# Suyashagarw/StreamOptima

Measured on AMD Instinct MI355X. Metric: encoded Mpixels/sec at 1080p & 4K, 1/2/4/8 GPUs; PSNR delta vs reference, higher is better.
Workload: dtype u8

## Files before the change

include/streamoptima.h:

```cpp
#ifndef STREAMOPTIMA_H
#define STREAMOPTIMA_H

#include <stddef.h>
#include <stdint.h>

#ifdef __cplusplus
extern "C" {
#endif

#define SO_OK 0
#define SO_E_INVALID (-1)
#define SO_E_UNSUPPORTED (-2)
#define SO_MAX_REF 4
#define SO_ABI_VERSION 1

int so_abi_version(void);
const char* so_last_error(void);

int so_me_full_search(const uint8_t* cur, const uint8_t* const* refs, int nref, int H,
                      int W, int bs, int sr, int32_t* out_best, int32_t* out_sub,
                      void* stream);

int so_inter_tq_recon(const uint8_t* cur, const uint8_t* const* refs, int nref, int H,
                      int W, int bs, const int32_t* best, const int32_t* sub, int qp_rd,
                      const int32_t* qp_row, int vbs, double lam, uint8_t* out_split,
                      int16_t* out_mv, int16_t* out_qtc, int32_t* out_tokens,
                      int32_t* out_mae_num, uint8_t* out_recon, int32_t* out_sse, void* stream);

size_t so_p_frame_scratch_elems(int H, int W, int bs, int vbs);

int so_encode_p_frame(const uint8_t* cur, const uint8_t* const* refs, int nref, int H,
                      int W, int bs, int sr, int qp_rd, const int32_t* qp_row, int vbs,
                      double lam, uint8_t* out_split, int16_t* out_mv, int16_t* out_qtc,
                      int32_t* out_tokens, int32_t* out_mae_num, uint8_t* out_recon,
                      int32_t* out_sse, int32_t* scratch, void* stream);

int so_encode_p_rows(const uint8_t* cur, const uint8_t* const* refs, int nref, int H, int W,
                     int bs, int sr, int by0, int by1, int qp_rd, const int32_t* qp_row,
                     int vbs, double lam, uint8_t* out_split, int16_t* out_mv,
                     int16_t* out_qtc, int32_t* out_tokens, int32_t* out_mae_num,
                     uint8_t* out_recon, int32_t* out_sse, int32_t* scratch, void* stream);

#define SO_OPT_RUN_2PASS_FUSED 1
#define SO_OPT_FASTME_SERIAL 2
#define SO_OPT_FASTME_SEGMENT 3
#define SO_OPT_FASTME_WARMUP 4
#define SO_OPT_COUNT_SAD_OPS 5
#define SO_OPT_TEST_LOSE_FLAG 6
#define SO_OPT_RUN_ZERO_SKIP 7
#define SO_OPT_RUN_TALL_TILES 8
int so_set_option(int option, int value);
int so_get_option(int option);

#define SO_P_RUN_TIMEOUT_WORD 32
#define SO_P_RUN_FALLBACK_WORD 64
#define SO_P_RUN_SAD_OPS_WORD 66
#define SO_P_RUN_TQ_FALLBACK_WORD 68
#define SO_P_RUN_STALE_WORD 33
#define SO_P_RUN_GAP_WORD 34
#define SO_P_RUN_DIAG_WORD 96
#define SO_P_RUN_DIAG_MAGIC 0x534F0001u
size_t so_p_run_workspace_elems(int H, int W);
int so_p_run_resident_workgroups(int vbs);
int so_p_run_mode_resident_workgroups(int mode, int vbs);
int so_p_run_tile_rows(int H, int W, int conc);
int so_encode_p_run(const uint8_t* const* curs, int nframes, const uint8_t* ref0, int H, int W,
                    int bs, int sr, int qp_rd, const int32_t* qp_row, int vbs, double lam,
                    uint8_t* const* out_split,
                    int16_t* const* out_mv, int16_t* const* out_qtc, int32_t* const* out_tokens,
                    int32_t* const* out_mae_num, uint8_t* const* out_recon, int32_t* const* out_sse,
                    uint32_t* workspace, void* stream);

int so_p_run_2pass_fused(int H, int W);

int so_encode_p_run_2pass(const uint8_t* const* curs, int nframes, const uint8_t* ref0, int H, int W,
                          int bs, int sr, int qp_rd, const int32_t* qp_row, const int32_t* roi,
                          int qp_lo, int qp_hi, uint8_t* const* out_split, int16_t* const* out_mv,
                          int16_t* const* out_qtc, int32_t* const* out_tokens,
                          int32_t* const* out_mae_num, uint8_t* const* out_recon,
                          int32_t* const* out_sse, int32_t* const* out_qp_map, uint32_t* workspace,
                          void* stream);

int so_encode_p_runs(const uint8_t* const* curs, int nframes, const uint8_t* const* refs,
// ... 273 lines not shown
```

streamoptima_amd/_lib.py:

```python
from __future__ import annotations

import ctypes
import os
import threading

import torch

from .build import LIB_PATH

_lock = threading.Lock()
_lib = None

SO_OK = 0
SO_E_INVALID = -1
SO_E_UNSUPPORTED = -2
MAX_REF = 4

_vp = ctypes.c_void_p
_i = ctypes.c_int
_d = ctypes.c_double
_sz = ctypes.c_size_t

_SIGS = {
    "so_abi_version": ([], _i),
# ... 79 lines not shown
    "so_pack_frames_huff": ([_i, _vp, _vp, _vp, _vp, _i, _i, _vp, _vp, ctypes.c_ulonglong, _vp, _vp], _i),
    "so_unpack_frames_huff": ([_i, _vp, _vp, _vp, _i, _i, _vp, _vp, _vp, _vp, _vp], _i),
    "so_pack_chroma_huff_bound": ([_i], _sz),
    "so_pack_chroma_frames_huff": ([_i, _vp, _vp, _i, _vp, _vp, ctypes.c_ulonglong, _vp, _vp], _i),
    "so_pack_chroma_frames_huff_after": ([_i, _vp, _vp, _i, _vp, _vp, _vp, ctypes.c_ulonglong, _vp, _vp], _i),
    "so_unpack_chroma_frames_huff": ([_i, _vp, _vp, _i, _vp, _vp, _vp, _vp], _i),
    "so_decode_p_frames": ([_i, _i, _vp, _vp, _i, _i, _i, _i, _vp, _vp, _vp, _i, _i, _vp, _vp, _vp, _vp, _vp], _i),
    "so_decode_chroma_frames": ([_i, _i, _vp, _vp, _vp, _i, _i, _i, _vp, _vp, _i, _vp, _vp, _i, _vp, _vp, _i, _i,
                                 _vp, _vp, _vp, _vp], _i),
    "so_decode_chroma_frames_ex": ([_i, _i, _vp, _vp, _vp, _i, _i, _i, _vp, _vp, _i, _vp, _vp, _i, _vp, _vp, _i, _i,
                                    _vp, _vp, _vp, _i, _vp], _i),
    "so_fme_plane_stride": ([_i, _i], _sz),
    "so_fme_workspace_bytes": ([_i, _i, _i], _sz),
    "so_fme_planes": ([_vp, _i, _i, _i, _vp, _vp], _i),
    "so_me_search_ex": ([_vp, _vp, _i, _i, _i, _i, _i, _i, _i, _i, _vp, _vp, _vp, _vp], _i),
    "so_encode_p_rows_ex": ([_vp, _vp, _i, _i, _i, _i, _i, _i, _i, _i, _vp, _vp, _i, _d, _i, _i, _i, _vp, _i,
                             _vp, _vp, _vp, _vp, _vp, _vp, _vp, _vp, _vp], _i),
    "so_inter_recon_ex": ([_vp, _i, _i, _i, _i, _i, _vp, _vp, _i, _i, _vp, _vp, _vp, _vp, _vp, _vp], _i),
    "so_encode_i_rows_ex": ([_vp, _i, _i, _i, _i, _i, _i, _i, _vp, _vp, _i, _d, _vp, _vp, _vp, _vp, _vp, _vp,
                             _vp, _vp, _vp], _i),
    "so_intra_recon_ex": ([_i, _i, _i, _i, _vp, _vp, _vp, _vp, _vp, _vp, _vp, _vp], _i),
    "so_qp_map": ([_vp, _i, _i, _i, _i, _i, _i, _vp, _vp, _i, _i, _vp, _vp], _i),
    "so_set_option": ([_i, _i], _i),
    "so_get_option": ([_i], _i),
}

ME_FULL, ME_FAST, ME_FAST_PAR = 0, 1, 2
REUSE_ME = 1
TOKENS_ONLY = 2
OPT_RUN_2PASS_FUSED, OPT_FASTME_SERIAL, OPT_FASTME_SEGMENT, OPT_FASTME_WARMUP, OPT_COUNT_SAD_OPS = 1, 2, 3, 4, 5
OPT_RUN_ZERO_SKIP = 7
OPT_RUN_TALL_TILES = 8
OPT_TEST_LOSE_FLAG = 6
COLOUR_MATRICES = {"bt601": 0, "bt709": 1}
COLOUR_LAYOUTS = {"hwc": 0, "chw": 1}

EXPORTED = tuple(_SIGS)


class HipPathError(RuntimeError):
    """Raised when the gfx950 library is unavailable or a kernel call fails."""


def load(path: str | None = None):
    global _lib
    with _lock:
        if _lib is not None:
            return _lib
        p = path or os.environ.get("SO_LIB_PATH") or LIB_PATH
        if not os.path.exists(p):
            raise HipPathError(
                f"{p} is missing: build it with `python -m streamoptima_amd.build` (hipcc, gfx950). "
                "There is no CPU fallback for the encode path.")
        lib = ctypes.CDLL(p)
        for name, (args, res) in _SIGS.items():
            if p != LIB_PATH and not hasattr(lib, name):
                continue
            fn = getattr(lib, name)
            fn.argtypes = args
            fn.restype = res
        if lib.so_abi_version() != 1:
            raise HipPathError("libstreamoptima_hip.so ABI mismatch")
        _lib = lib
        return lib


# ... 50 lines not shown
```

streamoptima_amd/csrc/so_capi.hip:

```cpp
#include <stdarg.h>
#include <stdio.h>
#include <stdlib.h>
#include <string.h>

#include <algorithm>
#include <atomic>
#include <vector>

#include <hip/hip_ext.h>

#include "so_chroma.h"
#include "so_colour.h"
#include "so_common.h"
#include "so_deblock.h"
#include "so_launch.h"
#include "so_packfmt.h"
#include "so_run.h"
#include "so_scale.h"

namespace so {

static thread_local char g_err[512] = "";

void set_error(const char* fmt, ...) {
    va_list ap;
    va_start(ap, fmt);
    vsnprintf(g_err, sizeof(g_err), fmt, ap);
    va_end(ap);
}

static std::atomic<int> g_opt[9] = {0, 1, 0, 32, 32, 0, 0, 0, -1};

int option(int id) {
    return (id > 0 && id < 9) ? g_opt[id].load(std::memory_order_relaxed) : 0;
}

#ifdef SO_AB
extern "C" int so_debug_ab_build(void) { return 1; }
#endif

static bool use_fused(int bs, int sr, int vbs, int nref) {
    if (bs != 16 || sr != 16 || vbs || nref != 1) return false;
#ifdef SO_AB
    const char* f = getenv("SO_FUSED");
    if (f && strcmp(f, "0") == 0) return false;
    const char* impl = getenv("SO_ME_IMPL");
    return impl == nullptr || impl[0] == 0;
#else
    return true;
#endif
}

static int check_vbs(const char* fn, int vbs, double lam) {
    if (vbs != 0 && vbs != 1) {
        set_error("%s: vbs must be 0 or 1", fn);
        return SO_E_INVALID;
    }
    if (vbs && !(lam >= 0.0 && lam < 1e300)) {
        set_error("%s: lambda %g (VBSEnable needs a finite lambda >= 0)", fn, lam);
        return SO_E_INVALID;
    }
    return SO_OK;
}

static int check_geom(const char* fn, int H, int W, int bs, int vbs) {
    if (bs != 16 && bs != 8) {
        set_error("%s: block_size %d not built (gfx950 kernels exist for 16 and 8)", fn, bs);
// ... 147 lines not shown
};

static int check_spans(const char* fn, std::vector<Span>& spans, bool dst_vs_dst) {
    std::sort(spans.begin(), spans.end(), [](const Span& a, const Span& b) { return a.lo < b.lo; });
    const Span *far_src = nullptr, *far_dst = nullptr;
    for (const Span& s : spans) {
        const Span* hit = nullptr;
        if (far_dst && s.lo < far_dst->hi && (!s.dst || dst_vs_dst)) hit = far_dst;
        if (!hit && s.dst && far_src && s.lo < far_src->hi) hit = far_src;
        if (hit) {
            set_error("%s: %s[%d] aliases %s[%d] (a destination overlaps a source or another destination)", fn,
                      s.what, s.frame, hit->what, hit->frame);
            return SO_E_INVALID;
        }
        const Span*& far = s.dst ? far_dst : far_src;
        if (!far || s.hi > far->hi) far = &s;
    }
    return SO_OK;
}

}

using namespace so;

extern "C" {

int so_abi_version(void) { return SO_ABI_VERSION; }

int so_set_option(int opt, int value) {
    const bool ok = (opt == SO_OPT_RUN_2PASS_FUSED || opt == SO_OPT_FASTME_SERIAL || opt == SO_OPT_COUNT_SAD_OPS ||
                     opt == SO_OPT_RUN_ZERO_SKIP)
                        ? (value == 0 || value == 1)
                    : opt == SO_OPT_RUN_TALL_TILES                               ? (value >= -1 && value <= 1)
                    : opt == SO_OPT_FASTME_SEGMENT                               ? value >= 1
                    : opt == SO_OPT_FASTME_WARMUP || opt == SO_OPT_TEST_LOSE_FLAG ? value >= 0
                                                                                 : false;
    if (!ok) {
        set_error("so_set_option: option %d value %d is unknown or out of range", opt, value);
        return SO_E_INVALID;
    }
    g_opt[opt].store(value, std::memory_order_relaxed);
    return SO_OK;
}

int so_get_option(int opt) { return option(opt); }

const char* so_last_error(void) { return g_err; }

int so_me_full_search(const uint8_t* cur, const uint8_t* const* refs, int nref, int H, int W, int bs,
                      int sr, int32_t* out_best, int32_t* out_sub, void* stream) {
    const char* fn = "so_me_full_search";
    SO_TRY(check_geom(fn, H, W, bs, out_sub != nullptr));
    SO_TRY(check_sr(fn, sr));
    SO_NEED(cur, fn);
    SO_NEED(out_best, fn);
    RefSet rs;
    SO_TRY(make_refs(fn, refs, nref, &rs));
    return me_launch(cur, rs, nref, H, W, bs, sr, 0, H / bs, out_best, out_sub, (hipStream_t)stream);
}

int so_inter_tq_recon(const uint8_t* cur, const uint8_t* const* refs, int nref, int H, int W, int bs,
                      const int32_t* best, const int32_t* sub, int qp_rd, const int32_t* qp_row, int vbs,
                      double lam, uint8_t* out_split, int16_t* out_mv, int16_t* out_qtc, int32_t* out_tokens,
                      int32_t* out_mae_num, uint8_t* out_recon, int32_t* out_sse, void* stream) {
    const char* fn = "so_inter_tq_recon";
    SO_TRY(check_geom(fn, H, W, bs, vbs));
// ... 1349 lines not shown
```

streamoptima_amd/csrc/so_intra.hip:

```cpp
#include "so_block.h"
#include "so_launch.h"

namespace so {

constexpr int kIntraMaxSr = 64;

SO_DEV uint32_t intra_key(int sad, int dx, int scan_rev) {
    return ((uint32_t)sad << 15) | ((uint32_t)(dx < 0 ? -dx : dx) << 8) | (uint32_t)scan_rev;
}

SO_DEV int canvas_at(const uint8_t* left , int sr, int col, int x0) {
    return col < x0 ? (int)left[col - (x0 - sr)] : 128;
}

template <int BS, bool VBS, int SRM = kIntraMaxSr>
__global__ void __launch_bounds__(256)
intra_tq_kernel(const uint8_t* __restrict__ cur, int H, int W, int by0, int nrows, int sr, int qp_rd,
                const int32_t* __restrict__ qp_row, const int32_t* __restrict__ qp_map, double lam,
                uint8_t* __restrict__ out_split,
                int16_t* __restrict__ out_mv, int16_t* __restrict__ out_qtc,
                int32_t* __restrict__ out_tokens, int32_t* __restrict__ out_mae,
                uint8_t* __restrict__ idres) {
    constexpr int G = BS, BPW = 256 / G, SB = BS / 2;
    constexpr int LDS_D = VBS ? 288 : BS * (BS + 1);
    __shared__ double ldsd[BPW * LDS_D];
    __shared__ uint8_t ldsf[VBS ? BPW * BS * BS : 1];
    __shared__ uint8_t ldsl[BPW * BS * SRM];
    const int tid = threadIdx.x, g = tid / G, l = tid % G;
    const int nbx = W / BS, nb = nbx * nrows;
    const int b = blockIdx.x * BPW + g;
    if (b >= nb) return;
    double* dl = ldsd + g * LDS_D;
    uint8_t* fl = ldsf + g * BS * BS;
    uint8_t* left = ldsl + g * BS * SRM;
    const int bx = b % nbx, by = by0 + b / nbx, x = bx * BS, y = by * BS;
    const int qpr = qp_map ? qp_map[(size_t)by * nbx + bx] : (qp_row ? qp_row[by] : qp_rd);

    uint8_t* lrow = left + l * SRM;
    if (BS == 16 && sr == 16 && x != 0) {
        *reinterpret_cast<uint4*>(lrow) = *reinterpret_cast<const uint4*>(cur + (size_t)(y + l) * W + x - 16);
    } else {
        for (int k = 0; k < sr; ++k) {
            const int col = x - sr + k;
            lrow[k] = col >= 0 ? cur[(size_t)(y + l) * W + col] : 0;
        }
    }
    int crow[BS];
    load_cur_row<BS>(cur, W, x, y + l, crow);
    wave_sync();

    int mv, sad;
    if (x == 0) {
        int s = 0;
#pragma unroll
        for (int c = 0; c < BS; ++c) s += abs(crow[c] - 128);
        sad = group_sum<G>(s);
        mv = -1;
    } else if (BS == 16 && sr == 16) {
        const uint8_t* rp = cur + (size_t)(y + l) * W + x;
        const uint4 lv = *reinterpret_cast<const uint4*>(rp - 16), cv = *reinterpret_cast<const uint4*>(rp);
        const uint32_t Z[9] = {lv.x, lv.y, lv.z, lv.w, 0x80808080u, 0x80808080u, 0x80808080u, 0x80808080u,
                               0x80808080u};
        const uint32_t C[4] = {cv.x, cv.y, cv.z, cv.w};
        uint32_t bestk = 0xFFFFFFFFu;
#pragma unroll
        for (int dx = -16; dx <= 0; ++dx) {
            const int off = 16 + dx, d = off >> 2, sh = off & 3;
            uint32_t srow = 0;
#pragma unroll
            for (int k = 0; k < 4; ++k)
                srow = __builtin_amdgcn_sad_u8(C[k], __builtin_amdgcn_alignbyte(Z[d + k + 1], Z[d + k], sh), srow);
            const int sfull = group_sum<G>((int)srow);
            const uint32_t key = ((uint32_t)sfull << 8) | (uint32_t)(-dx);
            bestk = key < bestk ? key : bestk;
        }
        sad = (int)(bestk >> 8);
        mv = -(int)(bestk & 0xFF);
    } else {
        uint32_t bestk = 0xFFFFFFFFu;
        for (int dxi = 0; dxi <= 2 * sr; ++dxi) {
            const int dx = dxi - sr;
            if (!(x + dx >= 0 && x + dx + BS <= W)) continue;
            int s = 0;
#pragma unroll
            for (int c = 0; c < BS; ++c) s += abs(crow[c] - canvas_at(lrow, sr, x + dx + c, x));
            s = group_sum<G>(s);
            const uint32_t k = intra_key(s, dx, 2 * sr - dxi);
            bestk = k < bestk ? k : bestk;
        }
        sad = (int)(bestk >> 15);
        mv = 2 * sr - (int)(bestk & 0xFF) - sr;
    }
    int res[BS];
#pragma unroll
    for (int c = 0; c < BS; ++c) res[c] = crow[c] - (x == 0 ? 128 : canvas_at(lrow, sr, x + mv + c, x));
    double tcd[BS];
    xform2d_rows<BS, false>(dl, l, res, tcd);
    int tc[BS], q[BS];
#pragma unroll
    for (int c = 0; c < BS; ++c) tc[c] = (int)__builtin_rint(tcd[c]);
    quant_row_i<BS>(tc, l, qp_rd, q);

    bool split = false;
    int mae_num = sad;
    const int j = l >> 2, r0 = l & 3;
    int smv = 0, stc[2][8], qs[2][8];
    if constexpr (VBS) {
        if (x != 0 && y != 0) {
            const int xs = x + (j & 1) * SB, oy = (j >> 1) * SB;
            int scur[2][8];
#pragma unroll
            for (int h = 0; h < 2; ++h) load_cur_row<8>(cur, W, xs, y + oy + r0 + 4 * h, scur[h]);
            int ssad;
            if (sr == 16) {
                uint32_t Zs[2][9], Cs[2][2];
#pragma unroll
                for (int h = 0; h < 2; ++h) {
                    const uint8_t* rp = cur + (size_t)(y + oy + r0 + 4 * h) * W + x;
                    const uint4 lv = *reinterpret_cast<const uint4*>(rp - 16);
                    const uint2 cv = *reinterpret_cast<const uint2*>(rp + (j & 1) * 8);
                    Zs[h][0] = lv.x; Zs[h][1] = lv.y; Zs[h][2] = lv.z; Zs[h][3] = lv.w;
                    Zs[h][4] = Zs[h][5] = Zs[h][6] = Zs[h][7] = Zs[h][8] = 0x80808080u;
                    Cs[h][0] = cv.x; Cs[h][1] = cv.y;
                }
                const int base = 16 + (j & 1) * 8;
                uint32_t bestk = 0xFFFFFFFFu;
#pragma unroll
                for (int dx = -16; dx <= 0; ++dx) {
                    const int off = base + dx;
                    const int d = off >> 2, sh = off & 3;
                    uint32_t srow = 0;
#pragma unroll
                    for (int h = 0; h < 2; ++h) {
                        uint32_t w0 = Zs[h][0], w1 = Zs[h][1], w2 = Zs[h][2];
// ... 31 lines not shown
                ssad = (int)(bestk >> 15);
                smv = 2 * sr - (int)(bestk & 0xFF) - sr;
            }
            int sres[2][8];
#pragma unroll
            for (int h = 0; h < 2; ++h) {
                const uint8_t* lr = left + (oy + r0 + 4 * h) * SRM;
#pragma unroll
                for (int c = 0; c < 8; ++c) sres[h][c] = scur[h][c] - canvas_at(lr, sr, xs + smv + c, x);
            }
            double std_[2][8];
            xform2d_sub<false>(dl, l, sres, std_);
            const int qpm1_rd = qp_rd > 0 ? qp_rd - 1 : qp_rd;
#pragma unroll
            for (int h = 0; h < 2; ++h) {
#pragma unroll
                for (int c = 0; c < 8; ++c) stc[h][c] = (int)__builtin_rint(std_[h][c]);
                quant_row<8>(stc[h], r0 + 4 * h, qpm1_rd, qs[h]);
            }
            const int tok_b = block_tokens<BS>(fl, l, q);
            const int tok_v = sub_tokens(fl, l, qs);
            int ssum = (r0 == 0) ? ssad : 0;
            ssum = group_sum<16>(ssum);
            const double mae_b = (double)sad / 256.0;
            const double mae_v = (double)ssum / 256.0;
            const double c_v = rd_cost(lam, 32 + 8 * tok_v, mae_v);
            const double c_b = rd_cost(lam, 8 + 8 * tok_b, mae_b);
            split = !(c_b < c_v);
            mae_num = ssum;
        }
    }

    int tok;
    uint8_t* rb = idres + (size_t)b * BS * BS;
    if (!split) {
        if (qpr != qp_rd) quant_row_i<BS>(tc, l, qpr, q);
        tok = block_tokens<BS>(fl, l, q);
        store_row_i16<BS>(out_qtc + (size_t)b * BS * BS + l * BS, q);
        int dq[BS];
        dequant_row_int<BS>(q, l, qpr, dq);
        double rd[BS];
        xform2d_rows<BS, true>(dl, l, dq, rd);
        int rr[BS];
#pragma unroll
        for (int c = 0; c < BS; ++c) rr[c] = (int)__builtin_rint(rd[c]);
        store_row_u8<BS>(rb, BS, 0, l, rr);
        for (int k = l; k < 4; k += G) out_mv[(size_t)b * 4 + k] = (int16_t)(k == 0 ? mv : 0);
    } else {
        if constexpr (VBS) {
            const int qpm1 = qpr > 0 ? qpr - 1 : qpr;
            const int qpm1_rd = qp_rd > 0 ? qp_rd - 1 : qp_rd;
            if (qpm1 != qpm1_rd)
#pragma unroll
                for (int h = 0; h < 2; ++h) quant_row<8>(stc[h], r0 + 4 * h, qpm1, qs[h]);
            tok = sub_tokens(fl, l, qs);
            int sdq[2][8];
#pragma unroll
            for (int h = 0; h < 2; ++h) {
                store_row_i16<8>(out_qtc + (size_t)b * BS * BS + j * 64 + (r0 + 4 * h) * 8, qs[h]);
                dequant_row<8>(qs[h], r0 + 4 * h, qpm1, sdq[h]);
            }
            double srd[2][8];
            xform2d_sub<true>(dl, l, sdq, srd);
#pragma unroll
            for (int h = 0; h < 2; ++h) {
                int rr[SB];
#pragma unroll
                for (int c = 0; c < SB; ++c) rr[c] = (int)__builtin_rint(srd[h][c]);
                store_row_u8<SB>(rb, BS, (j & 1) * SB, (j >> 1) * SB + r0 + 4 * h, rr);
            }
            if (r0 == 0) out_mv[(size_t)b * 4 + j] = (int16_t)smv;
        } else {
            tok = 0;
        }
    }
    if (l == 0) {
        out_split[b] = (uint8_t)split;
        out_tokens[b] = tok;
        out_mae[b] = mae_num;
    }
}

template <int BS, bool VBS>
__global__ void __launch_bounds__(256)
dequant_idct_kernel(int H, int W, int qp, const int32_t* __restrict__ qp_row, const int32_t* __restrict__ qp_map,
                    const uint8_t* __restrict__ split, const int16_t* __restrict__ qtc,
                    uint8_t* __restrict__ idres) {
    constexpr int G = BS, BPW = 256 / G;
    constexpr int LDS_D = VBS ? 288 : BS * (BS + 1);
    __shared__ double ldsd[BPW * LDS_D];
    const int tid = threadIdx.x, g = tid / G, l = tid % G;
    const int nbx = W / BS, nb = nbx * (H / BS);
    const int b = blockIdx.x * BPW + g;
    if (b >= nb) return;
    double* dl = ldsd + g * LDS_D;
    const int by = b / nbx;
    const int qpr = qp_map ? qp_map[b] : (qp_row ? qp_row[by] : qp);
    uint8_t* rb = idres + (size_t)b * BS * BS;
    if (!VBS || !split[b]) {
        int q[BS], dq[BS];
        load_row_i16<BS>(qtc + (size_t)b * BS * BS + l * BS, q);
        dequant_row<BS>(q, l, qpr, dq);
        double rd[BS];
        xform2d_rows<BS, true>(dl, l, dq, rd);
        int rr[BS];
#pragma unroll
        for (int c = 0; c < BS; ++c) rr[c] = (int)__builtin_rint(rd[c]);
        store_row_u8<BS>(rb, BS, 0, l, rr);
    } else if constexpr (VBS) {
        const int j = l >> 2, r0 = l & 3;
        const int qpm1 = qpr > 0 ? qpr - 1 : qpr;
        int sdq[2][8];
// ... 147 lines not shown
            const int bx = bx0 + s;
            if (bx < nbx) {
                const int x = bx * BS;
                int v = resc[s] + 128;
                const int src = x + c + dxc[s];
                if (x != 0 && src < x) v = resc[s] + vr[src & (RING - 1)];
                vr[(x + c) & (RING - 1)] = v;
                const int o = v & 255;
                if (act) {
                    orow[x + c] = (uint8_t)o;
                    const int d = curc[s] - o;
                    sse += d * d;
                }
            }
        }
    }
    if (out_sse) {
#pragma unroll
        for (int m = BS / 2; m >= 1; m >>= 1) sse += __shfl_xor(sse, m, 64);
        if (act && c == 0) out_sse[yl] = sse;
    }
}

template <int BS, int WPR>
__global__ void __launch_bounds__(64 * WPR)
intra_recon_scan_kernel(int W, int nrows_px, int by0, const uint8_t* __restrict__ split, const int16_t* __restrict__ mv,
                        const uint8_t* __restrict__ idres, const uint8_t* __restrict__ cur,
                        uint8_t* __restrict__ out_recon, int32_t* __restrict__ out_sse) {
    constexpr int NT = 64 * WPR, K = NT / BS, GPW = 64 / BS, SB = BS / 2, ND = BS / 4, TU = 4, U3 = 4;
    extern __shared__ __attribute__((aligned(16))) uint16_t slot[];
    __shared__ int ssum[WPR];
    const int tid = threadIdx.x, lane = tid & 63, wv = tid >> 6;
    const int k = tid / BS, c = tid - k * BS, g = k - wv * GPW;
    const int xcd = blockIdx.x & 7, kx = blockIdx.x >> 3;
    const int yl = (((kx / BS) << 3) + xcd) * BS + kx % BS;
    if (yl >= nrows_px) return;
    const int yy = by0 * BS + yl, byl = yl / BS, i = yl - byl * BS, nbx = W / BS;
    const int L = (nbx + K - 1) / K, j0 = k * L;
    const bool lower = i >= SB;
    uint32_t* const ev = reinterpret_cast<uint32_t*>(slot + (size_t)L * NT);
    uint8_t* const rowb = reinterpret_cast<uint8_t*>(ev + NT);
    for (int t0 = 0; t0 * NT < nbx; t0 += TU) {
        uint32_t rw[TU][ND], mw[TU][2], sp[TU];
#pragma unroll
        for (int t = 0; t < TU; ++t) {
            int jb = (t0 + t) * NT + tid;
            jb = jb < nbx ? jb : nbx - 1;
            const size_t b = (size_t)byl * nbx + jb;
            const uint32_t* rp = reinterpret_cast<const uint32_t*>(idres + b * BS * BS + i * BS);
#pragma unroll
            for (int d = 0; d < ND; ++d) rw[t][d] = rp[d];
            const uint2 m4 = *reinterpret_cast<const uint2*>(mv + b * 4);
            mw[t][0] = m4.x;
            mw[t][1] = m4.y;
            sp[t] = split[b];
        }
#pragma unroll
        for (int t = 0; t < TU; ++t) {
            const int jb = (t0 + t) * NT + tid;
            if (jb < nbx) {
                const uint32_t wlr = (sp[t] && lower) ? mw[t][1] : mw[t][0];
                const int dxl = (int)(int16_t)(wlr & 0xFFFF);
                const int dxr = sp[t] ? (int)(int16_t)(wlr >> 16) : dxl;
                const int kq = jb / L, s = jb - kq * L;
                uint32_t pk[BS / 2];
#pragma unroll
                for (int cc = 0; cc < BS; ++cc) {
                    const int rel = cc + (cc >= SB ? dxr : dxl);
                    const bool use = jb != 0 && rel < 0;
                    const uint32_t v = ((rw[t][cc >> 2] >> (8 * (cc & 3))) & 255u) | (use ? 256u : 0u) |
                                       ((uint32_t)((rel + BS) & (BS - 1)) << 9);
                    pk[cc >> 1] = (cc & 1) ? (pk[cc >> 1] | (v << 16)) : v;
                }
                uint4* dst = reinterpret_cast<uint4*>(slot + (size_t)s * NT + kq * BS);
#pragma unroll
                for (int q = 0; q < BS / 8; ++q) dst[q] = make_uint4(pk[4 * q], pk[4 * q + 1], pk[4 * q + 2], pk[4 * q + 3]);
            }
        }
    }
    __syncthreads();
    const int gbase = lane & ~(BS - 1);
    const int nvalid = nbx - j0 < L ? (nbx - j0 > 0 ? nbx - j0 : 0) : L;
    uint32_t w = (uint32_t)(c + 1) << 8;
    uint32_t in = slot[tid];
    for (int s = 0; s < nvalid; ++s) {
        const uint32_t cin = in;
        if (s + 1 < nvalid) in = slot[(s + 1) * NT + tid];
        const uint32_t gv = (uint32_t)__builtin_amdgcn_ds_bpermute((gbase + (int)(cin >> 9)) << 2, (int)w);
        const bool use = (cin & 256u) != 0u;
        w = ((cin + (use ? gv : 128u)) & 255u) | (use ? (gv & 0x1F00u) : 0u);
        slot[s * NT + tid] = (uint16_t)w;
    }
    uint32_t P = w;
#pragma unroll
    for (int gg = 1; gg < GPW; ++gg) {
        const uint32_t si = (w >> 8) & 31u;
        const uint32_t pg = (uint32_t)__builtin_amdgcn_ds_bpermute(((gg - 1) * BS + (int)(si ? si - 1 : 0)) << 2, (int)P);
        if (g == gg) P = ((w + (si ? pg : 0u)) & 255u) | (si ? (pg & 0x1F00u) : 0u);
    }
#pragma unroll
    for (int ww = 0; ww < WPR; ++ww) {
        if (wv == ww) {
            const uint32_t si = (P >> 8) & 31u;
            const uint32_t e = (ww > 0 && si) ? ev[(ww * GPW - 1) * BS + si - 1] : 0u;
            ev[tid] = (P + e) & 255u;
        }
        __syncthreads();
    }
    const uint32_t* const ein = ev + (k > 0 ? k - 1 : 0) * BS - 1;
    for (int s0 = 0; s0 < nvalid; s0 += U3) {
        uint32_t m[U3];
#pragma unroll
        for (int u = 0; u < U3; ++u) m[u] = s0 + u < nvalid ? slot[(s0 + u) * NT + tid] : 0u;
#pragma unroll
        for (int u = 0; u < U3; ++u) {
// ... 5 lines not shown
    __syncthreads();
    const uint8_t* crow = cur ? cur + (size_t)yy * W : nullptr;
    uint8_t* orow = out_recon + (size_t)yy * W;
    int sse = 0;
    for (int x0 = tid * 16; x0 < W; x0 += NT * 16) {
        const uint4 r = *reinterpret_cast<const uint4*>(rowb + x0);
        *reinterpret_cast<uint4*>(orow + x0) = r;
        if (crow) {
            const uint4 q = *reinterpret_cast<const uint4*>(crow + x0);
            const uint32_t rr[4] = {r.x, r.y, r.z, r.w}, qq[4] = {q.x, q.y, q.z, q.w};
#pragma unroll
            for (int d = 0; d < 4; ++d)
#pragma unroll
                for (int e = 0; e < 4; ++e) {
                    const int df = (int)((qq[d] >> (8 * e)) & 255u) - (int)((rr[d] >> (8 * e)) & 255u);
                    sse += df * df;
                }
        }
    }
    if (out_sse) {
#pragma unroll
        for (int m = 32; m >= 1; m >>= 1) sse += __shfl_xor(sse, m, 64);
        if (lane == 0) ssum[wv] = sse;
        __syncthreads();
        if (tid == 0) {
            int t = 0;
#pragma unroll
            for (int ww = 0; ww < WPR; ++ww) t += ssum[ww];
            out_sse[yl] = t;
        }
    }
}

constexpr int kIrsWpr = 4;
constexpr int kIrsWpb = 1;
static int intra_recon_rows(int W, int bs, int sr, int by0, int nrows_px, const uint8_t* split, const int16_t* mv,
                            const uint8_t* idres, const uint8_t* cur, uint8_t* out_recon, int32_t* out_sse, int H,
                            hipStream_t st) {
    if (nrows_px <= 0) return SO_OK;
    const bool a16 = ((reinterpret_cast<uintptr_t>(cur) | reinterpret_cast<uintptr_t>(out_recon)) & 15) == 0;
    if (sr <= bs && W % 16 == 0 && a16) {
        constexpr int WPR = kIrsWpr, NT = 64 * WPR;
        const int k = NT / bs, nbx = W / bs, L = (nbx + k - 1) / k;
        const size_t lds = (size_t)L * NT * sizeof(uint16_t) + NT * sizeof(uint32_t) + (size_t)W;
        const int nbr = (nrows_px + bs - 1) / bs, grid = (nbr + 7) / 8 * 8 * bs;
        if (bs == 16)
            hipLaunchKernelGGL((intra_recon_scan_kernel<16, WPR>), dim3(grid), dim3(NT), lds, st, W, nrows_px, by0,
                               split, mv, idres, cur, out_recon, out_sse);
        else
            hipLaunchKernelGGL((intra_recon_scan_kernel<8, WPR>), dim3(grid), dim3(NT), lds, st, W, nrows_px, by0,
                               split, mv, idres, cur, out_recon, out_sse);
        return check_launch("intra_recon_scan_kernel");
    }
    if (sr <= 64) {
        const int rows_per_blk = kIrsWpb * (64 / bs);
        const dim3 grid((nrows_px + rows_per_blk - 1) / rows_per_blk);
#define SO_IRS(B, N)                                                                                              \
    hipLaunchKernelGGL((intra_recon_seq_kernel<B, N>), grid, dim3(64 * kIrsWpb), 0, st, W, nrows_px, by0, split, \
                       mv, idres, cur, out_recon, out_sse)
        if (bs == 16) { if (sr <= 16) SO_IRS(16, true); else SO_IRS(16, false); }
        else { if (sr <= 8) SO_IRS(8, true); else SO_IRS(8, false); }
#undef SO_IRS
        return check_launch("intra_recon_seq_kernel");
    }
    if (bs == 16)
        hipLaunchKernelGGL((intra_recon_kernel<16>), dim3(nrows_px), dim3(256), 12 * (size_t)W, st, H, W, by0, split,
                           mv, idres, cur, out_recon, out_sse);
    else
        hipLaunchKernelGGL((intra_recon_kernel<8>), dim3(nrows_px), dim3(256), 12 * (size_t)W, st, H, W, by0, split,
                           mv, idres, cur, out_recon, out_sse);
    return check_launch("intra_recon_kernel");
}

int intra_encode_launch(const uint8_t* cur, int H, int W, int bs, int sr, int by0, int by1, int qp_rd,
                        const int32_t* qp_row, const int32_t* qp_map, int vbs, double lam, uint8_t* out_split, int16_t* out_mv,
                        int16_t* out_qtc, int32_t* out_tokens, int32_t* out_mae, uint8_t* out_recon,
                        int32_t* out_sse, uint8_t* idres, hipStream_t st) {
    const int nrows = by1 - by0;
    if (nrows <= 0) return SO_OK;
    const int nb = (W / bs) * nrows;
    const int bpw = 256 / bs;
    dim3 grid((nb + bpw - 1) / bpw), blk(256);
    if (bs == 16 && vbs)
        hipLaunchKernelGGL((intra_tq_kernel<16, true>), grid, blk, 0, st, cur, H, W, by0, nrows, sr, qp_rd, qp_row, qp_map,
// ... 38 lines not shown
```

Before: 190,300.

## Specialize 16x16 intra TQ path and auto-pick scan waves per row

For the non-VBS 16x16 intra kernel, the row search is rewritten to compute all offsets with packed SAD instructions and DPP row sums. The left-row staging buffer is removed and aliased onto the transform scratch, and the transform switches to a dword-pitched variant. Quantisation and dequantisation become exponent bit tricks driven by DPP, with an occupancy hint of 8 waves per EU. Separately, the intra recon scan kernel now chooses 2, 3 or 4 waves per row from a cached occupancy query and a cost model, with an option to override. This adds complexity and risks exact-rounding differences in the fast quant path.

```diff
diff --git a/include/streamoptima.h b/include/streamoptima.h
--- a/include/streamoptima.h
+++ b/include/streamoptima.h
@@ -49,6 +49,7 @@
 #define SO_OPT_TEST_LOSE_FLAG 6
 #define SO_OPT_RUN_ZERO_SKIP 7
 #define SO_OPT_RUN_TALL_TILES 8
+#define SO_OPT_INTRA_SCAN_WAVES 9
 int so_set_option(int option, int value);
 int so_get_option(int option);
 
diff --git a/streamoptima_amd/_lib.py b/streamoptima_amd/_lib.py
--- a/streamoptima_amd/_lib.py
+++ b/streamoptima_amd/_lib.py
@@ -135,6 +135,7 @@
 OPT_RUN_ZERO_SKIP = 7
 OPT_RUN_TALL_TILES = 8
 OPT_TEST_LOSE_FLAG = 6
+OPT_INTRA_SCAN_WAVES = 9
 COLOUR_MATRICES = {"bt601": 0, "bt709": 1}
 COLOUR_LAYOUTS = {"hwc": 0, "chw": 1}
 
diff --git a/streamoptima_amd/csrc/so_capi.hip b/streamoptima_amd/csrc/so_capi.hip
--- a/streamoptima_amd/csrc/so_capi.hip
+++ b/streamoptima_amd/csrc/so_capi.hip
@@ -29,10 +29,10 @@
     va_end(ap);
 }
 
-static std::atomic<int> g_opt[9] = {0, 1, 0, 32, 32, 0, 0, 0, -1};
+static std::atomic<int> g_opt[10] = {0, 1, 0, 32, 32, 0, 0, 0, -1, 0};
 
 int option(int id) {
-    return (id > 0 && id < 9) ? g_opt[id].load(std::memory_order_relaxed) : 0;
+    return (id > 0 && id < 10) ? g_opt[id].load(std::memory_order_relaxed) : 0;
 }
 
 #ifdef SO_AB
@@ -246,6 +246,7 @@
                      opt == SO_OPT_RUN_ZERO_SKIP)
                         ? (value == 0 || value == 1)
                     : opt == SO_OPT_RUN_TALL_TILES                               ? (value >= -1 && value <= 1)
+                    : opt == SO_OPT_INTRA_SCAN_WAVES                             ? (value == 0 || (value >= 2 && value <= 4))
                     : opt == SO_OPT_FASTME_SEGMENT                               ? value >= 1
                     : opt == SO_OPT_FASTME_WARMUP || opt == SO_OPT_TEST_LOSE_FLAG ? value >= 0
                                                                                  : false;
diff --git a/streamoptima_amd/csrc/so_intra.hip b/streamoptima_amd/csrc/so_intra.hip
--- a/streamoptima_amd/csrc/so_intra.hip
+++ b/streamoptima_amd/csrc/so_intra.hip
@@ -1,4 +1,9 @@
+#include <map>
+#include <mutex>
+#include <tuple>
+
 #include "so_block.h"
+#include "so_intra_map.h"
 #include "so_launch.h"
 
 namespace so {
@@ -9,12 +14,22 @@
     return ((uint32_t)sad << 15) | ((uint32_t)(dx < 0 ? -dx : dx) << 8) | (uint32_t)scan_rev;
 }
 
+template <int G, bool ROW>
+SO_DEV int intra_group_sum(int v) {
+    if constexpr (ROW) {
+        static_assert(G == 16, "a DPP row is 16 lanes");
+        return (int)row_sum_u32((uint32_t)v);
+    } else {
+        return group_sum<G>(v);
+    }
+}
+
 SO_DEV int canvas_at(const uint8_t* left , int sr, int col, int x0) {
     return col < x0 ? (int)left[col - (x0 - sr)] : 128;
 }
 
 template <int BS, bool VBS, int SRM = kIntraMaxSr>
-__global__ void __launch_bounds__(256)
+__global__ void __launch_bounds__(256) __attribute__((amdgpu_waves_per_eu((BS == 16 && !VBS) ? 8 : 1)))
 intra_tq_kernel(const uint8_t* __restrict__ cur, int H, int W, int by0, int nrows, int sr, int qp_rd,
                 const int32_t* __restrict__ qp_row, const int32_t* __restrict__ qp_map, double lam,
                 uint8_t* __restrict__ out_split,
@@ -22,21 +37,88 @@
                 int32_t* __restrict__ out_tokens, int32_t* __restrict__ out_mae,
                 uint8_t* __restrict__ idres) {
     constexpr int G = BS, BPW = 256 / G, SB = BS / 2;
-    constexpr int LDS_D = VBS ? 288 : BS * (BS + 1);
+    constexpr bool DW = BS == 16 && !VBS;
+    constexpr int LDS_D = VBS ? 288 : (DW ? 136 : BS * (BS + 1));
     __shared__ double ldsd[BPW * LDS_D];
     __shared__ uint8_t ldsf[VBS ? BPW * BS * BS : 1];
-    __shared__ uint8_t ldsl[BPW * BS * SRM];
-    const int tid = threadIdx.x, g = tid / G, l = tid % G;
+    __shared__ uint8_t ldsl[DW ? 1 : BPW * BS * SRM];
+    static_assert(!DW || BS * SRM <= LDS_D * (int)sizeof(double), "the left pixels fit the block's scratch");
+    const int tid = threadIdx.x;
+    int g = tid / G, l = tid % G;
     const int nbx = W / BS, nb = nbx * nrows;
-    const int b = blockIdx.x * BPW + g;
+    int b = blockIdx.x * BPW + g;
     if (b >= nb) return;
     double* dl = ldsd + g * LDS_D;
     uint8_t* fl = ldsf + g * BS * BS;
-    uint8_t* left = ldsl + g * BS * SRM;
+    uint8_t* left = DW ? reinterpret_cast<uint8_t*>(dl) : ldsl + g * BS * SRM;
+    static_assert(!DW || LDS_D * 2 == imap::kDwBlock, "xform2d_rows_dw: 16 x 17 dwords per block");
     const int bx = b % nbx, by = by0 + b / nbx, x = bx * BS, y = by * BS;
-    const int qpr = qp_map ? qp_map[(size_t)by * nbx + bx] : (qp_row ? qp_row[by] : qp_rd);
+    int qpr = qp_map ? qp_map[(size_t)by * nbx + bx] : (qp_row ? qp_row[by] : qp_rd);
+    const auto derive = [&]() {
+        if constexpr (DW) {
+            int t = (int)threadIdx.x;
+            asm volatile("" : "+v"(t));
+            g = t / G;
+            l = t % G;
+            b = (int)blockIdx.x * BPW + g;
+            dl = ldsd + g * LDS_D;
+            qpr = qp_map ? qp_map[(size_t)by0 * nbx + b] : (qp_row ? qp_row[by0 + b / nbx] : qp_rd);
+        }
+    };
 
     uint8_t* lrow = left + l * SRM;
+    int mv, sad, res[BS];
+    if (DW && sr == 16) {
+        constexpr uint32_t F = 0x80808080u;
+        const uint8_t* rp = cur + (size_t)(y + l) * W + x;
+        const uint4 cv = *reinterpret_cast<const uint4*>(rp);
+        const uint32_t C[4] = {cv.x, cv.y, cv.z, cv.w};
+        uint32_t sfill[5];
+        sfill[4] = 0;
+#pragma unroll
+        for (int k = 3; k >= 0; --k) sfill[k] = __builtin_amdgcn_sad_u8(C[k], F, sfill[k + 1]);
+        uint32_t P[4] = {F, F, F, F};
+        if (x == 0) {
+            sad = (int)row_sum_u32(sfill[0]);
+            mv = -1;
+        } else {
+            const uint4 lv = *reinterpret_cast<const uint4*>(rp - 16);
+            const uint32_t Z[5] = {lv.x, lv.y, lv.z, lv.w, F};
+            uint32_t srow[17];
+#pragma unroll
+            for (int off = 0; off <= 16; ++off) {
+                const int d = off >> 2, sh = off & 3;
+                uint32_t s = sfill[4 - d];
+#pragma unroll
+                for (int k = 0; k < 4 - d; ++k)
+                    s = __builtin_amdgcn_sad_u8(C[k], __builtin_amdgcn_alignbyte(Z[d + k + 1], Z[d + k], sh), s);
+                srow[off] = s;
+            }
+            uint32_t bestk = 0xFFFFFFFFu;
+#pragma unroll
+            for (int off = 0; off < 16; off += 2) {
+                const uint32_t two = row_sum_u32(srow[off] | (srow[off + 1] << 16));
+                const uint32_t k0 = ((two & 0xFFFFu) << 8) | (uint32_t)(16 - off);
+                const uint32_t k1 = ((two >> 16) << 8) | (uint32_t)(15 - off);
+                bestk = k0 < bestk ? k0 : bestk;
+                bestk = k1 < bestk ? k1 : bestk;
+            }
+            const uint32_t k16 = row_sum_u32(srow[16]) << 8;
+            bestk = k16 < bestk ? k16 : bestk;
+            sad = (int)(bestk >> 8);
+            mv = -(int)(bestk & 0xFF);
+            const uint32_t off = (uint32_t)(16 + mv), sh = off & 3u;
+            uint32_t D[5] = {Z[0], Z[1], Z[2], Z[3], F};
+            if (off & 4u) { D[0] = D[1]; D[1] = D[2]; D[2] = D[3]; D[3] = F; }
+            if (off & 8u) { D[0] = D[2]; D[1] = D[3]; D[2] = F; D[3] = F; }
+            if (off & 16u) { D[0] = F; D[1] = F; D[2] = F; D[3] = F; }
+#pragma unroll
+            for (int k = 0; k < 4; ++k) P[k] = __builtin_amdgcn_alignbyte(D[k + 1], D[k], sh);
+        }
+#pragma unroll
+        for (int c = 0; c < BS; ++c)
+            res[c] = (int)((C[(c >> 2) & 3] >> (8 * (c & 3))) & 255u) - (int)((P[(c >> 2) & 3] >> (8 * (c & 3))) & 255u);
+    } else {
     if (BS == 16 && sr == 16 && x != 0) {
         *reinterpret_cast<uint4*>(lrow) = *reinterpret_cast<const uint4*>(cur + (size_t)(y + l) * W + x - 16);
     } else {
@@ -49,12 +131,11 @@
     load_cur_row<BS>(cur, W, x, y + l, crow);
     wave_sync();
 
-    int mv, sad;
     if (x == 0) {
         int s = 0;
 #pragma unroll
         for (int c = 0; c < BS; ++c) s += abs(crow[c] - 128);
-        sad = group_sum<G>(s);
+        sad = intra_group_sum<G, DW>(s);
         mv = -1;
     } else if (BS == 16 && sr == 16) {
         const uint8_t* rp = cur + (size_t)(y + l) * W + x;
@@ -70,7 +151,7 @@
 #pragma unroll
             for (int k = 0; k < 4; ++k)
                 srow = __builtin_amdgcn_sad_u8(C[k], __builtin_amdgcn_alignbyte(Z[d + k + 1], Z[d + k], sh), srow);
-            const int sfull = group_sum<G>((int)srow);
+            const int sfull = intra_group_sum<G, DW>((int)srow);
             const uint32_t key = ((uint32_t)sfull << 8) | (uint32_t)(-dx);
             bestk = key < bestk ? key : bestk;
         }
@@ -84,22 +165,44 @@
             int s = 0;
 #pragma unroll
             for (int c = 0; c < BS; ++c) s += abs(crow[c] - canvas_at(lrow, sr, x + dx + c, x));
-            s = group_sum<G>(s);
+            s = intra_group_sum<G, DW>(s);
             const uint32_t k = intra_key(s, dx, 2 * sr - dxi);
             bestk = k < bestk ? k : bestk;
         }
         sad = (int)(bestk >> 15);
         mv = 2 * sr - (int)(bestk & 0xFF) - sr;
     }
-    int res[BS];
 #pragma unroll
     for (int c = 0; c < BS; ++c) res[c] = crow[c] - (x == 0 ? 128 : canvas_at(lrow, sr, x + mv + c, x));
+    if constexpr (DW) wave_sync();
+    }
+    if constexpr (DW) {
+        if (l < 4) out_mv[(size_t)b * 4 + l] = (int16_t)(l == 0 ? mv : 0);
+        if (l == 0) {
+            out_split[b] = 0;
+            out_mae[b] = sad;
+        }
+    }
     double tcd[BS];
-    xform2d_rows<BS, false>(dl, l, res, tcd);
+    if constexpr (DW) xform2d_rows_dw<false>(dl, l, res, tcd, typename dct::Rfft<16>::TW{});
+    else xform2d_rows<BS, false>(dl, l, res, tcd);
     int tc[BS], q[BS];
-#pragma unroll
-    for (int c = 0; c < BS; ++c) tc[c] = (int)__builtin_rint(tcd[c]);
-    quant_row_i<BS>(tc, l, qp_rd, q);
+    derive();
+    if constexpr (DW) {
+        constexpr double kRne = 0x1.8p52;
+        const int sc_hi2 = (1023 - 2 - qpr) << 20;
+        int sc_hi = (1023 - qpr - (l == 15 ? 1 : 0)) << 20;
+#pragma unroll
+        for (int c = 0; c < BS; ++c) {
+            const double sc = __builtin_bit_cast(double, (uint64_t)(uint32_t)sc_hi << 32);
+            q[c] = (int)(uint32_t)__builtin_bit_cast(uint64_t, __builtin_fma(__builtin_rint(tcd[c]), sc, kRne));
+            if (c < BS - 1) sc_hi = __builtin_amdgcn_update_dpp(sc_hi2, sc_hi, 0x101, 0xF, 0xF, false);
+        }
+    } else {
+#pragma unroll
+        for (int c = 0; c < BS; ++c) tc[c] = (int)__builtin_rint(tcd[c]);
+        quant_row_i<BS>(tc, l, qp_rd, q);
+    }
 
     bool split = false;
     int mae_num = sad;
@@ -197,20 +300,35 @@
     }
 
     int tok;
-    uint8_t* rb = idres + (size_t)b * BS * BS;
     if (!split) {
-        if (qpr != qp_rd) quant_row_i<BS>(tc, l, qpr, q);
-        tok = block_tokens<BS>(fl, l, q);
+        if constexpr (!DW)
+            if (qpr != qp_rd) quant_row_i<BS>(tc, l, qpr, q);
+        tok = block_tokens<BS, DW>(fl, l, q);
         store_row_i16<BS>(out_qtc + (size_t)b * BS * BS + l * BS, q);
         int dq[BS];
-        dequant_row_int<BS>(q, l, qpr, dq);
+        if constexpr (DW) {
+            int k = qpr + (l == 15 ? 1 : 0);
+#pragma unroll
+            for (int c = 0; c < BS; ++c) {
+                dq[c] = (int)((uint32_t)q[c] << k);
+                if (c < BS - 1) k = __builtin_amdgcn_update_dpp(qpr + 2, k, 0x101, 0xF, 0xF, false);
+            }
+        } else {
+            dequant_row_int<BS>(q, l, qpr, dq);
+        }
         double rd[BS];
-        xform2d_rows<BS, true>(dl, l, dq, rd);
+        if constexpr (DW) xform2d_rows_dw<true>(dl, l, dq, rd, typename dct::Rfft<16>::TW{});
+        else xform2d_rows<BS, true>(dl, l, dq, rd);
+        derive();
         int rr[BS];
 #pragma unroll
-        for (int c = 0; c < BS; ++c) rr[c] = (int)__builtin_rint(rd[c]);
-        store_row_u8<BS>(rb, BS, 0, l, rr);
-        for (int k = l; k < 4; k += G) out_mv[(size_t)b * 4 + k] = (int16_t)(k == 0 ? mv : 0);
+        for (int c = 0; c < BS; ++c) {
+            if constexpr (DW) rr[c] = (int)(uint32_t)__builtin_bit_cast(uint64_t, rd[c] + 0x1.8p52);
+            else rr[c] = (int)__builtin_rint(rd[c]);
+        }
+        store_row_u8<BS>(idres + (size_t)b * BS * BS, BS, 0, l, rr);
+        if constexpr (!DW)
+            for (int k = l; k < 4; k += G) out_mv[(size_t)b * 4 + k] = (int16_t)(k == 0 ? mv : 0);
     } else {
         if constexpr (VBS) {
             const int qpm1 = qpr > 0 ? qpr - 1 : qpr;
@@ -232,7 +350,7 @@
                 int rr[SB];
 #pragma unroll
                 for (int c = 0; c < SB; ++c) rr[c] = (int)__builtin_rint(srd[h][c]);
-                store_row_u8<SB>(rb, BS, (j & 1) * SB, (j >> 1) * SB + r0 + 4 * h, rr);
+                store_row_u8<SB>(idres + (size_t)b * BS * BS, BS, (j & 1) * SB, (j >> 1) * SB + r0 + 4 * h, rr);
             }
             if (r0 == 0) out_mv[(size_t)b * 4 + j] = (int16_t)smv;
         } else {
@@ -240,9 +358,11 @@
         }
     }
     if (l == 0) {
-        out_split[b] = (uint8_t)split;
         out_tokens[b] = tok;
-        out_mae[b] = mae_num;
+        if constexpr (!DW) {
+            out_split[b] = (uint8_t)split;
+            out_mae[b] = mae_num;
+        }
     }
 }
 
@@ -456,11 +576,10 @@
     __shared__ int ssum[WPR];
     const int tid = threadIdx.x, lane = tid & 63, wv = tid >> 6;
     const int k = tid / BS, c = tid - k * BS, g = k - wv * GPW;
-    const int xcd = blockIdx.x & 7, kx = blockIdx.x >> 3;
-    const int yl = (((kx / BS) << 3) + xcd) * BS + kx % BS;
+    const int yl = imap::scan_row_of((int)blockIdx.x, BS);
     if (yl >= nrows_px) return;
     const int yy = by0 * BS + yl, byl = yl / BS, i = yl - byl * BS, nbx = W / BS;
-    const int L = (nbx + K - 1) / K, j0 = k * L;
+    const int L = imap::scan_chunk_len(nbx, BS, WPR), j0 = k * L;
     const bool lower = i >= SB;
     uint32_t* const ev = reinterpret_cast<uint32_t*>(slot + (size_t)L * NT);
     uint8_t* const rowb = reinterpret_cast<uint8_t*>(ev + NT);
@@ -486,7 +605,7 @@
                 const uint32_t wlr = (sp[t] && lower) ? mw[t][1] : mw[t][0];
                 const int dxl = (int)(int16_t)(wlr & 0xFFFF);
                 const int dxr = sp[t] ? (int)(int16_t)(wlr >> 16) : dxl;
-                const int kq = jb / L, s = jb - kq * L;
+                const int kq = imap::scan_chunk_of(jb, L), s = jb - kq * L;
                 uint32_t pk[BS / 2];
 #pragma unroll
                 for (int cc = 0; cc < BS; ++cc) {
@@ -504,7 +623,7 @@
     }
     __syncthreads();
     const int gbase = lane & ~(BS - 1);
-    const int nvalid = nbx - j0 < L ? (nbx - j0 > 0 ? nbx - j0 : 0) : L;
+    const int nvalid = imap::scan_chunk_valid(nbx, k, L);
     uint32_t w = (uint32_t)(c + 1) << 8;
     uint32_t in = slot[tid];
     for (int s = 0; s < nvalid; ++s) {
@@ -576,7 +695,30 @@
     }
 }
 
-constexpr int kIrsWpr = 4;
+static int scan_resident(const void* kernel, int nt, size_t lds) {
+    static std::mutex mu;
+    static std::map<std::tuple<int, const void*, size_t>, int> cache;
+    int dev = 0;
+    if (hipGetDevice(&dev) != hipSuccess) return 0;
+    std::lock_guard<std::mutex> lk(mu);
+    const auto key = std::make_tuple(dev, kernel, lds);
+    auto it = cache.find(key);
+    if (it == cache.end()) {
+        int n = 0, p = 0;
+        if (hipDeviceGetAttribute(&n, hipDeviceAttributeMultiprocessorCount, dev) != hipSuccess || n <= 0) n = 0;
+        if (hipOccupancyMaxActiveBlocksPerMultiprocessor(&p, kernel, nt, lds) != hipSuccess || p <= 0) p = 0;
+        it = cache.emplace(key, n * p).first;
+    }
+    return it->second;
+}
+
+template <int BS>
+static const void* scan_kernel_of(int wpr) {
+    return wpr == 2 ? reinterpret_cast<const void*>(&intra_recon_scan_kernel<BS, 2>)
+         : wpr == 3 ? reinterpret_cast<const void*>(&intra_recon_scan_kernel<BS, 3>)
+                    : reinterpret_cast<const void*>(&intra_recon_scan_kernel<BS, 4>);
+}
+
 constexpr int kIrsWpb = 1;
 static int intra_recon_rows(int W, int bs, int sr, int by0, int nrows_px, const uint8_t* split, const int16_t* mv,
                             const uint8_t* idres, const uint8_t* cur, uint8_t* out_recon, int32_t* out_sse, int H,
@@ -584,16 +726,23 @@
     if (nrows_px <= 0) return SO_OK;
     const bool a16 = ((reinterpret_cast<uintptr_t>(cur) | reinterpret_cast<uintptr_t>(out_recon)) & 15) == 0;
     if (sr <= bs && W % 16 == 0 && a16) {
-        constexpr int WPR = kIrsWpr, NT = 64 * WPR;
-        const int k = NT / bs, nbx = W / bs, L = (nbx + k - 1) / k;
-        const size_t lds = (size_t)L * NT * sizeof(uint16_t) + NT * sizeof(uint32_t) + (size_t)W;
-        const int nbr = (nrows_px + bs - 1) / bs, grid = (nbr + 7) / 8 * 8 * bs;
-        if (bs == 16)
-            hipLaunchKernelGGL((intra_recon_scan_kernel<16, WPR>), dim3(grid), dim3(NT), lds, st, W, nrows_px, by0,
-                               split, mv, idres, cur, out_recon, out_sse);
-        else
-            hipLaunchKernelGGL((intra_recon_scan_kernel<8, WPR>), dim3(grid), dim3(NT), lds, st, W, nrows_px, by0,
-                               split, mv, idres, cur, out_recon, out_sse);
+        const int nbx = W / bs;
+        int wpr = option(SO_OPT_INTRA_SCAN_WAVES);
+        if (wpr < imap::kScanWprMin || wpr > imap::kScanWprMax) {
+            int res[imap::kScanWprMax - imap::kScanWprMin + 1];
+            for (int w = imap::kScanWprMin; w <= imap::kScanWprMax; ++w)
+                res[w - imap::kScanWprMin] = scan_resident(bs == 16 ? scan_kernel_of<16>(w) : scan_kernel_of<8>(w),
+                                                           imap::scan_threads(w), imap::scan_lds_bytes(W, bs, w));
+            wpr = imap::scan_pick_wpr(nbx, bs, nrows_px, res);
+        }
+        const size_t lds = imap::scan_lds_bytes(W, bs, wpr);
+        const int grid = imap::scan_grid(nrows_px, bs);
+#define SO_SCAN(B, N)                                                                                              \
+    hipLaunchKernelGGL((intra_recon_scan_kernel<B, N>), dim3(grid), dim3(64 * N), lds, st, W, nrows_px, by0, split, \
+                       mv, idres, cur, out_recon, out_sse)
+        if (bs == 16) { if (wpr == 2) SO_SCAN(16, 2); else if (wpr == 3) SO_SCAN(16, 3); else SO_SCAN(16, 4); }
+        else { if (wpr == 2) SO_SCAN(8, 2); else if (wpr == 3) SO_SCAN(8, 3); else SO_SCAN(8, 4); }
+#undef SO_SCAN
         return check_launch("intra_recon_scan_kernel");
     }
     if (sr <= 64) {
diff --git a/streamoptima_amd/csrc/so_intra_map.h b/streamoptima_amd/csrc/so_intra_map.h
--- /dev/null
+++ b/streamoptima_amd/csrc/so_intra_map.h
@@ -0,0 +1,57 @@
+#pragma once
+#include <cstddef>
+#include <cstdint>
+
+namespace so {
+namespace imap {
+
+#if defined(__HIPCC__)
+#define SO_IMAP_FN __host__ __device__ constexpr
+#else
+#define SO_IMAP_FN constexpr
+#endif
+
+SO_IMAP_FN int scan_threads(int wpr) { return 64 * wpr; }
+SO_IMAP_FN int scan_chunks(int bs, int wpr) { return scan_threads(wpr) / bs; }
+SO_IMAP_FN int scan_chunk_len(int nbx, int bs, int wpr) {
+    return (nbx + scan_chunks(bs, wpr) - 1) / scan_chunks(bs, wpr);
+}
+SO_IMAP_FN int scan_chunk_of(int jb, int L) { return jb / L; }
+SO_IMAP_FN int scan_step_of(int jb, int L) { return jb % L; }
+SO_IMAP_FN int scan_chunk_valid(int nbx, int k, int L) {
+    return nbx - k * L < L ? (nbx - k * L > 0 ? nbx - k * L : 0) : L;
+}
+SO_IMAP_FN size_t scan_slot(int s, int t, int wpr) { return (size_t)s * scan_threads(wpr) + t; }
+SO_IMAP_FN size_t scan_lds_bytes(int W, int bs, int wpr) {
+    return (size_t)scan_chunk_len(W / bs, bs, wpr) * scan_threads(wpr) * sizeof(uint16_t) +
+           (size_t)scan_threads(wpr) * sizeof(uint32_t) + (size_t)W;
+}
+SO_IMAP_FN int scan_row_of(int wg, int bs) {
+    return ((((wg >> 3) / bs) << 3) + (wg & 7)) * bs + (wg >> 3) % bs;
+}
+SO_IMAP_FN int scan_grid(int nrows_px, int bs) { return ((nrows_px + bs - 1) / bs + 7) / 8 * 8 * bs; }
+
+SO_IMAP_FN long scan_cost(int nbx, int bs, int wpr, int nrows_px, int resident) {
+    const int r = resident > 0 ? resident : 1;
+    return (long)((nrows_px + r - 1) / r) * (scan_chunk_len(nbx, bs, wpr) + 64 / bs + wpr);
+}
+constexpr int kScanWprMin = 2, kScanWprMax = 4;
+SO_IMAP_FN int scan_pick_wpr(int nbx, int bs, int nrows_px, const int* resident) {
+    int best = kScanWprMax;
+    long bc = scan_cost(nbx, bs, kScanWprMax, nrows_px, resident[kScanWprMax - kScanWprMin]);
+    for (int w = kScanWprMax - 1; w >= kScanWprMin; --w) {
+        const long c = scan_cost(nbx, bs, w, nrows_px, resident[w - kScanWprMin]);
+        if (c < bc) { bc = c; best = w; }
+    }
+    return best;
+}
+
+constexpr int kDwPitch = 17, kDwBlock = 16 * kDwPitch;
+SO_IMAP_FN int dw_block_base(int g) { return g * kDwBlock; }
+SO_IMAP_FN int dw_row_elem(int l, int c) { return l * kDwPitch + c; }
+SO_IMAP_FN int dw_col_elem(int l, int r) { return r * kDwPitch + l; }
+
+#undef SO_IMAP_FN
+
+}
+}
```

After: 191,200, median of 6. No clear change (+0.5%).
